# niessner/BundleFusion

Measured on AMD Instinct MI355X. Metric: frames/sec end-to-end (SIFT+SBA+TSDF re-integrate), 640x480 @4mm, higher is better.
Workload: dtype f32

## Files before the change

### bundlefusion_amd/csrc/solver.hip

```cpp
#include <hip/hip_runtime.h>

#include <algorithm>
#include <cstring>
#include <vector>

#include "bf_device.h"
#include "bf_resources.h"
#include "bf_se3.h"

using namespace bf;

namespace {

constexpr float FLOAT_EPSILON = 0.000001f;
constexpr uint32_t NOSLOT = 0xFFFFFFFFu;
constexpr int DENSE_BLK = 120;

typedef float f32x4 __attribute__((ext_vector_type(4)));

enum Flag { FL_DONE = 0, FL_NUM_SLOTS = 1, FL_NUM_PAIRS = 2, FL_LIST_LEN = 3, FL_GN_ITERS = 4, FL_BARRIER_FAIL = 5, FL_SLOT_OVERFLOW = 6, FL_PCG_ITERS = 8, FL_COUNT = 40 };

struct Cfg {
    float denseDistThresh, denseNormalThresh, denseColorThresh, denseColorGradientMin, denseDepthMin, denseDepthMax;
    uint32_t subsample;
// ... 523 lines not shown
            d.slotG[(size_t)s * 6 + (lane - 36)] = c.wSparse * accD + dD;
        } else if (lane < 46) {
            d.slotP[(size_t)s * 4 + (lane - 42)] = accD;
        }
    }
}

__global__ __launch_bounds__(256) void k_rows(Dev d) {
    if (d.flags[FL_DONE]) return;
    const uint32_t lane = threadIdx.x & 63;
    const uint32_t i = blockIdx.x * (blockDim.x >> 6) + (threadIdx.x >> 6);
    if (i >= d.N) return;
    const uint32_t s0 = d.rowStart[i], s1 = d.rowStart[i + 1];
    float acc = 0.0f;
    for (uint32_t s = s0; s < s1; ++s) {
        if (lane < 36) acc += d.slotD[(size_t)s * 36 + lane];
        else if (lane < 42) acc += d.slotG[(size_t)s * 6 + (lane - 36)];
        else if (lane < 46) acc += d.slotP[(size_t)s * 4 + (lane - 42)];
    }
    if (lane < 36) d.diagA[(size_t)i * 36 + lane] = acc;
    else if (lane < 42) d.rhs[(size_t)i * 6 + (lane - 36)] = -acc;
    else if (lane < 45) d.prec[(size_t)i * 6 + 3 + (lane - 42)] = acc > FLOAT_EPSILON ? 1.0f / acc : 1.0f;
    else if (lane == 45) {
        const float v = acc > FLOAT_EPSILON ? 1.0f / acc : 1.0f;
        d.prec[(size_t)i * 6 + 0] = v; d.prec[(size_t)i * 6 + 1] = v; d.prec[(size_t)i * 6 + 2] = v;
    }
}

BF_DEV float blockSum(float v, float* sh) {
    v = wave_sum(v);
    __syncthreads();
    if ((threadIdx.x & 63) == 0) sh[threadIdx.x >> 6] = v;
    __syncthreads();
    float t = 0.0f;
    for (uint32_t w = 0; w < (blockDim.x >> 6); ++w) t += sh[w];
    return t;
}
BF_DEV float blockMax(float v, float* sh) {
    v = wave_max(v);
    __syncthreads();
    if ((threadIdx.x & 63) == 0) sh[threadIdx.x >> 6] = v;
    __syncthreads();
    float t = 0.0f;
    for (uint32_t w = 0; w < (blockDim.x >> 6); ++w) t = fmaxf(t, sh[w]);
    return t;
}

constexpr size_t PCG_LDS_MAX = 160 * 1024 - 1024;
template <bool VEC_LDS>
__global__ __launch_bounds__(1024) void k_pcg(Dev d, uint32_t nLin, uint32_t gnIter, int lastGN) {
    if (d.flags[FL_DONE]) return;
    extern __shared__ float dynLds[];
    __shared__ float sh[16];
    const uint32_t N = d.N, n6 = 6 * N;
    const uint32_t lane = threadIdx.x & 63, wave = threadIdx.x >> 6, nWaves = blockDim.x >> 6;
    float* const P = VEC_LDS ? dynLds : d.p;
    float* const R = VEC_LDS ? dynLds + n6 : d.r;
    float* const X = VEC_LDS ? dynLds + 2 * n6 : d.delta;
    float* const AP = VEC_LDS ? dynLds + 3 * n6 : d.Ap;
    const float* const M = VEC_LDS ? dynLds + 4 * n6 : d.prec;
    const uint32_t* const RS = VEC_LDS ? (const uint32_t*)(dynLds + 5 * n6) : d.rowStart;
    if (VEC_LDS) {
        for (uint32_t t = threadIdx.x; t < n6; t += blockDim.x) dynLds[4 * n6 + t] = d.prec[t];
        for (uint32_t t = threadIdx.x; t <= N; t += blockDim.x) ((uint32_t*)(dynLds + 5 * n6))[t] = d.rowStart[t];
        __syncthreads();
    }
    float part = 0.0f;
    for (uint32_t t = threadIdx.x; t < n6; t += blockDim.x) {
        const bool var = t >= 6;
        const float rr = var ? d.rhs[t] : 0.0f;
        const float pp = var ? M[t] * rr : 0.0f;
        R[t] = rr; P[t] = pp; X[t] = 0.0f;
        part += rr * pp;
    }
    float rzOld = blockSum(part, sh);
    uint32_t it = 0;
    for (uint32_t lin = 0; lin < nLin; ++lin) {
        bool last = (lin == nLin - 1);
        ++it;
        __syncthreads();
        {
            const uint32_t q = lane >> 4, l16 = lane & 15;
            for (uint32_t i0 = 1; i0 < N; i0 += 4 * nWaves) {
                const uint32_t i = i0 + wave * 4 + q;
                float acc[6] = {0, 0, 0, 0, 0, 0};
                if (i < N) {
                    const uint32_t s0 = RS[i], s1 = RS[i + 1];
                    for (uint32_t s = s0 + l16; s < s1; s += 16) {
                        const float4* O4 = reinterpret_cast<const float4*>(d.slotO + (size_t)s * 36);
                        const uint32_t col = d.slotCol[s];
                        float O[36];
#pragma unroll
                        for (int v = 0; v < 9; ++v) { const float4 o = O4[v]; O[4 * v] = o.x; O[4 * v + 1] = o.y; O[4 * v + 2] = o.z; O[4 * v + 3] = o.w; }
                        const float* pj = P + 6 * col;
                        const float q0 = pj[0], q1 = pj[1], q2 = pj[2], q3 = pj[3], q4 = pj[4], q5 = pj[5];
#pragma unroll
                        for (int a = 0; a < 6; ++a)
                            acc[a] += ((((O[a * 6 + 0] * q0 + O[a * 6 + 1] * q1) + O[a * 6 + 2] * q2) + O[a * 6 + 3] * q3) + O[a * 6 + 4] * q4) + O[a * 6 + 5] * q5;
                    }
                }
#pragma unroll
                for (int a = 0; a < 6; ++a)
#pragma unroll
                    for (int o = 8; o > 0; o >>= 1) acc[a] += __shfl_xor(acc[a], o, 64);
                if (i < N && l16 < 6) {
                    const float* A = d.diagA + (size_t)i * 36 + l16 * 6;
                    const float* pi = P + 6 * i;
                    float v = 0.0f;
#pragma unroll
                    for (int b = 0; b < 6; ++b) v += A[b] * pi[b];
                    float sel = acc[0];
                    if (l16 == 1) sel = acc[1]; else if (l16 == 2) sel = acc[2]; else if (l16 == 3) sel = acc[3]; else if (l16 == 4) sel = acc[4]; else if (l16 == 5) sel = acc[5];
                    AP[6 * i + l16] = v + sel;
                }
            }
        }
        __syncthreads();
        part = 0.0f;
        for (uint32_t t = 6 + threadIdx.x; t < n6; t += blockDim.x) part += P[t] * AP[t];
        const float pAp = blockSum(part, sh);
        const float alpha = pAp > FLOAT_EPSILON ? rzOld / pAp : 0.0f;
        part = 0.0f;
        for (uint32_t t = 6 + threadIdx.x; t < n6; t += blockDim.x) {
            X[t] = X[t] + alpha * P[t];
            const float rr = R[t] - alpha * AP[t];
            R[t] = rr;
            part += (M[t] * rr) * rr;
        }
        const float rzNew = blockSum(part, sh);
        if (fabsf(pAp) < 5e-7f) last = true;
        const float beta = rzOld > FLOAT_EPSILON ? rzNew / rzOld : 0.0f;
        rzOld = rzNew;
        for (uint32_t t = 6 + threadIdx.x; t < n6; t += blockDim.x) P[t] = M[t] * R[t] + beta * P[t];
        if (last) break;
    }
    __syncthreads();
    float mx = 0.0f;
    for (uint32_t i = 1 + threadIdx.x; i < N; i += blockDim.x) {
        const f3 dT = ld3(X + 6 * i), dW = ld3(X + 6 * i + 3);
        f3 nw, nt;
        lieUpdate(dW, dT, ld3(d.xRot + 3 * i), ld3(d.xTrans + 3 * i), nw, nt);
        d.xRot[3 * i] = nw.x; d.xRot[3 * i + 1] = nw.y; d.xRot[3 * i + 2] = nw.z;
        d.xTrans[3 * i] = nt.x; d.xTrans[3 * i + 1] = nt.y; d.xTrans[3 * i + 2] = nt.z;
        if (d.valid[i] != 0) mx = fmaxf(mx, fmaxf(fmaxf(fmaxf(fabsf(dW.x), fabsf(dT.x)), fmaxf(fabsf(dW.y), fabsf(dT.y))), fmaxf(fabsf(dW.z), fabsf(dT.z))));
    }
    mx = blockMax(mx, sh);
    if (threadIdx.x == 0) {
        d.flags[FL_GN_ITERS] = (int)gnIter + 1;
        d.flags[FL_PCG_ITERS + gnIter] = (int)it;
        if (!lastGN && mx < 0.005f) d.flags[FL_DONE] = 1;
    }
}

constexpr uint32_t COOP_THREADS = 256, COOP_THREADS_SMALL = 1024, COOP_MAX_GROUPS = 64, COOP_ROWS_PER_GROUP = 8, COOP_SPIN_LIMIT = 1u << 22;

BF_DEV void coopPublish(float* p, float v) { __hip_atomic_store(p, v, __ATOMIC_RELAXED, __HIP_MEMORY_SCOPE_AGENT); }
BF_DEV float coopRead(const float* p) { return __hip_atomic_load(p, __ATOMIC_RELAXED, __HIP_MEMORY_SCOPE_AGENT); }

BF_DEV bool gridBarrier(uint32_t* counter, uint32_t target, int* shFail) {
    __builtin_amdgcn_s_waitcnt(0);
    __syncthreads();
    if (threadIdx.x == 0) {
        __hip_atomic_fetch_add(counter, 1u, __ATOMIC_RELAXED, __HIP_MEMORY_SCOPE_AGENT);
        uint32_t spins = 0;
        while (__hip_atomic_load(counter, __ATOMIC_RELAXED, __HIP_MEMORY_SCOPE_AGENT) < target) {
            __builtin_amdgcn_s_sleep(2);
            if (++spins > COOP_SPIN_LIMIT) { *shFail = 1; break; }
        }
    }
    __syncthreads();
    return *shFail == 0;
}

template <uint32_t THREADS>
__global__ __launch_bounds__(THREADS) void k_pcg_coop(Dev d, uint32_t nLin, uint32_t gnIter, int lastGN, uint32_t ldsFloats, uint32_t vecGlobal) {
    if (d.flags[FL_DONE]) return;
    extern __shared__ __align__(16) float coopLds[];
    float* const dynLds = coopLds;
    __shared__ float sh[16];
    __shared__ int shFail;
    const uint32_t N = d.N, n6 = 6 * N, G = gridDim.x;
    const uint32_t lane = threadIdx.x & 63, wave = threadIdx.x >> 6, nWaves = THREADS >> 6;
    const uint32_t vecFloats = (5 * n6 + (N + 1) + 3) & ~3u;
    float* const vec = vecGlobal ? d.coopVec + (size_t)blockIdx.x * vecFloats : dynLds;
    float* const P = vec;
    float* const R = vec + n6;
    float* const X = vec + 2 * n6;
    float* const AP = vec + 3 * n6;
    float* const M = vec + 4 * n6;
    uint32_t* const RS = reinterpret_cast<uint32_t*>(vec + 5 * n6);
    const uint32_t rpg = (N - 1 + G - 1) / G;
    const uint32_t r0 = min(N, 1 + blockIdx.x * rpg), r1 = min(N, r0 + rpg);
    const uint32_t ldsBase = vecGlobal ? 0u : 5 * n6 + (N + 1);
    float* const DG = dynLds + ldsBase;
    float* const OL = dynLds + ((ldsBase + rpg * 36 + 3) & ~3u);
    if (threadIdx.x == 0) shFail = 0;
    for (uint32_t t = threadIdx.x; t < n6; t += THREADS) M[t] = d.prec[t];
    for (uint32_t t = threadIdx.x; t <= N; t += THREADS) RS[t] = d.rowStart[t];
    for (uint32_t t = threadIdx.x; t < (r1 - r0) * 36; t += THREADS) DG[t] = d.diagA[(size_t)r0 * 36 + t];
    __syncthreads();
    const uint32_t sBase = RS[r0], sEnd = RS[r1];
    const uint32_t ldsSlots = min(sEnd - sBase, (ldsFloats - (uint32_t)(OL - dynLds)) / 37u);
    uint32_t* const CL = reinterpret_cast<uint32_t*>(OL + (size_t)ldsSlots * 36);
    {
        const float4* src = reinterpret_cast<const float4*>(d.slotO + (size_t)sBase * 36);
        float4* dst = reinterpret_cast<float4*>(OL);
        for (uint32_t t = threadIdx.x; t < ldsSlots * 9; t += THREADS) dst[t] = src[t];
        for (uint32_t t = threadIdx.x; t < ldsSlots; t += THREADS) CL[t] = d.slotCol[sBase + t];
    }
    float part = 0.0f;
    for (uint32_t t = threadIdx.x; t < n6; t += THREADS) {
        const bool var = t >= 6;
        const float rr = var ? d.rhs[t] : 0.0f;
        const float pp = var ? M[t] * rr : 0.0f;
        R[t] = rr; P[t] = pp; X[t] = 0.0f;
        part += rr * pp;
    }
    float rzOld = blockSum(part, sh);
    float* const xchg[2] = {d.Ap, d.p};
    uint32_t* const counter = reinterpret_cast<uint32_t*>(d.gridBar) + gnIter;
    uint32_t it = 0;
    for (uint32_t lin = 0; lin < nLin; ++lin) {
        bool last = (lin == nLin - 1);
        ++it;
        __syncthreads();
        float* const out = G > 1 ? xchg[lin & 1] : AP;
        {
            const uint32_t g8 = lane >> 3, a = lane & 7;
            for (uint32_t i = r0 + wave; i < r1; i += nWaves) {
                const uint32_t s0 = RS[i], s1 = RS[i + 1];
                float acc = 0.0f;
                if (a < 6) {
                    for (uint32_t s = s0 + g8; s < s1; s += 8) {
                        const uint32_t ls = s - sBase;
                        float o0, o1, o2, o3, o4, o5; uint32_t col;
                        if (ls < ldsSlots) {
                            const float* O = OL + (size_t)ls * 36 + a * 6;
                            o0 = O[0]; o1 = O[1]; o2 = O[2]; o3 = O[3]; o4 = O[4]; o5 = O[5]; col = CL[ls];
                        } else {
                            const float* O = d.slotO + (size_t)s * 36 + a * 6;
                            o0 = O[0]; o1 = O[1]; o2 = O[2]; o3 = O[3]; o4 = O[4]; o5 = O[5]; col = d.slotCol[s];
                        }
                        const float* pj = P + 6 * col;
                        acc += ((((o0 * pj[0] + o1 * pj[1]) + o2 * pj[2]) + o3 * pj[3]) + o4 * pj[4]) + o5 * pj[5];
                    }
                }
                acc += __shfl_xor(acc, 8, 64); acc += __shfl_xor(acc, 16, 64); acc += __shfl_xor(acc, 32, 64);
                if (lane < 6) {
                    const float* A = DG + (size_t)(i - r0) * 36 + lane * 6;
                    const float* pi = P + 6 * i;
                    float v = 0.0f;
#pragma unroll
                    for (int b = 0; b < 6; ++b) v += A[b] * pi[b];
                    if (G > 1) coopPublish(out + 6 * i + lane, v + acc); else out[6 * i + lane] = v + acc;
                }
            }
        }
        part = 0.0f;
        if (G > 1) {
            if (!gridBarrier(counter, G * it, &shFail)) { if (threadIdx.x == 0) d.flags[FL_BARRIER_FAIL] = 1; return; }
            for (uint32_t t = 6 + threadIdx.x; t < n6; t += THREADS) { const float ap = coopRead(out + t); AP[t] = ap; part += P[t] * ap; }
        } else {
            __syncthreads();
            for (uint32_t t = 6 + threadIdx.x; t < n6; t += THREADS) part += P[t] * AP[t];
        }
        const float pAp = blockSum(part, sh);
        const float alpha = pAp > FLOAT_EPSILON ? rzOld / pAp : 0.0f;
        part = 0.0f;
        for (uint32_t t = 6 + threadIdx.x; t < n6; t += THREADS) {
            X[t] = X[t] + alpha * P[t];
            const float rr = R[t] - alpha * AP[t];
            R[t] = rr;
            part += (M[t] * rr) * rr;
        }
        const float rzNew = blockSum(part, sh);
        if (fabsf(pAp) < 5e-7f) last = true;
        const float beta = rzOld > FLOAT_EPSILON ? rzNew / rzOld : 0.0f;
        rzOld = rzNew;
        for (uint32_t t = 6 + threadIdx.x; t < n6; t += THREADS) P[t] = M[t] * R[t] + beta * P[t];
        if (last) break;
    }
    if (blockIdx.x != 0) return;
    __syncthreads();
    float mx = 0.0f;
    for (uint32_t i = 1 + threadIdx.x; i < N; i += THREADS) {
        const f3 dT = ld3(X + 6 * i), dW = ld3(X + 6 * i + 3);
        f3 nw, nt;
        lieUpdate(dW, dT, ld3(d.xRot + 3 * i), ld3(d.xTrans + 3 * i), nw, nt);
        d.xRot[3 * i] = nw.x; d.xRot[3 * i + 1] = nw.y; d.xRot[3 * i + 2] = nw.z;
        d.xTrans[3 * i] = nt.x; d.xTrans[3 * i + 1] = nt.y; d.xTrans[3 * i + 2] = nt.z;
        if (d.valid[i] != 0) mx = fmaxf(mx, fmaxf(fmaxf(fmaxf(fabsf(dW.x), fabsf(dT.x)), fmaxf(fabsf(dW.y), fabsf(dT.y))), fmaxf(fabsf(dW.z), fabsf(dT.z))));
    }
    mx = blockMax(mx, sh);
    if (threadIdx.x == 0) {
        d.flags[FL_GN_ITERS] = (int)gnIter + 1;
        d.flags[FL_PCG_ITERS + gnIter] = (int)it;
        if (!lastGN && mx < 0.005f) d.flags[FL_DONE] = 1;
    }
}

BF_DEV float absMaxResidual(const Dev& d, const bf_entry_j& e, float w) {
    if (!validCorr(e)) return 0.0f;
    const m44 TI = poseToMatrix(ld3(d.xRot + 3 * e.imgIdx_i), ld3(d.xTrans + 3 * e.imgIdx_i));
    const m44 TJ = poseToMatrix(ld3(d.xRot + 3 * e.imgIdx_j), ld3(d.xTrans + 3 * e.imgIdx_j));
    const f3 a = xform(TI, mk3(e.pos_i[0], e.pos_i[1], e.pos_i[2])), b = xform(TJ, mk3(e.pos_j[0], e.pos_j[1], e.pos_j[2]));
    return fmaxf(w * fabsf(a.z - b.z), fmaxf(w * fabsf(a.x - b.x), w * fabsf(a.y - b.y)));
}

constexpr uint32_t MAXRES_GROUPS = 64;
BF_DEV bool maxResBetter(float o, int oi, float cur, int ci) { return cur < o || (cur == o && oi < ci && o > 0.0f); }

__global__ __launch_bounds__(1024) void k_max_residual(Dev d, float w) {
    __shared__ float sv[1024];
    __shared__ int si[1024];
    float best = 0.0f; int bi = 0;
    for (uint32_t c = blockIdx.x * blockDim.x + threadIdx.x; c < d.C; c += gridDim.x * blockDim.x) {
        const float r = absMaxResidual(d, d.corr[c], w);
        if (best < r) { best = r; bi = (int)c; }
    }
    sv[threadIdx.x] = best; si[threadIdx.x] = bi;
    __syncthreads();
    for (uint32_t s = blockDim.x >> 1; s > 0; s >>= 1) {
        if (threadIdx.x < s) {
            const float o = sv[threadIdx.x + s]; const int oi = si[threadIdx.x + s];
            if (maxResBetter(o, oi, sv[threadIdx.x], si[threadIdx.x])) { sv[threadIdx.x] = o; si[threadIdx.x] = oi; }
        }
        __syncthreads();
    }
    if (threadIdx.x == 0) { d.maxResPart[blockIdx.x] = sv[0]; d.maxIdxPart[blockIdx.x] = si[0]; }
}

__global__ __launch_bounds__(64) void k_max_residual_final(Dev d, uint32_t G) {
    float best = 0.0f; int bi = 0;
    if (threadIdx.x < G) { best = d.maxResPart[threadIdx.x]; bi = d.maxIdxPart[threadIdx.x]; }
#pragma unroll
    for (int o = 32; o > 0; o >>= 1) {
        const float ov = __shfl_xor(best, o, 64); const int oi = __shfl_xor(bi, o, 64);
        if (maxResBetter(ov, oi, best, bi)) { best = ov; bi = oi; }
    }
    if (threadIdx.x == 0) { d.maxRes[0] = best; d.maxIdx[0] = bi; }
}

__global__ void k_count_high(Dev d, float w, float thresh) {
    const uint32_t c = blockIdx.x * blockDim.x + threadIdx.x;
    bool hi = false;
    if (c < d.C) hi = absMaxResidual(d, d.corr[c], w) > thresh;
    const unsigned long long m = __ballot(hi);
    if ((threadIdx.x & 63) == 0 && m) atomicAdd(d.highCount, __popcll(m));
}

__global__ __launch_bounds__(1024) void k_energy(Dev d, float w, uint32_t slot, int honourDone) {
    if (honourDone && d.flags[FL_DONE] && slot > (uint32_t)d.flags[FL_GN_ITERS]) return;
    __shared__ float sh[16];
    float part = 0.0f;
    for (uint32_t c = threadIdx.x; c < d.C; c += blockDim.x) {
        const bf_entry_j e = d.corr[c];
        if (!validCorr(e)) continue;
        const m44 TI = poseToMatrix(ld3(d.xRot + 3 * e.imgIdx_i), ld3(d.xTrans + 3 * e.imgIdx_i));
        const m44 TJ = poseToMatrix(ld3(d.xRot + 3 * e.imgIdx_j), ld3(d.xTrans + 3 * e.imgIdx_j));
        const f3 r = xform(TI, mk3(e.pos_i[0], e.pos_i[1], e.pos_i[2])) - xform(TJ, mk3(e.pos_j[0], e.pos_j[1], e.pos_j[2]));
        part += w * dot3(r, r);
    }
    const float tot = blockSum(part, sh);
    if (threadIdx.x == 0) d.energies[slot] = tot;
}

__global__ void k_matrices_to_poses(const m44* T, uint32_t n, float* rot3, float* trans3, const int* valid) {
    const uint32_t i = blockIdx.x * blockDim.x + threadIdx.x;
    if (i < n && valid[i]) {
        f3 r, t;
        matrixToPose(T[i], r, t);
        rot3[3 * i] = r.x; rot3[3 * i + 1] = r.y; rot3[3 * i + 2] = r.z;
        trans3[3 * i] = t.x; trans3[3 * i + 1] = t.y; trans3[3 * i + 2] = t.z;
    }
}
__global__ void k_poses_to_matrices(const float* rot3, const float* trans3, uint32_t n, m44* T, const int* valid) {
    const uint32_t i = blockIdx.x * blockDim.x + threadIdx.x;
    if (i < n && valid[i]) T[i] = poseToMatrix(ld3(rot3 + 3 * i), ld3(trans3 + 3 * i));
}

__global__ void k_expand_dense(Dev d, float* JtJ, float* Jtr) {
    const uint32_t nPairs = (uint32_t)d.flags[FL_NUM_PAIRS];
    const uint32_t dim = 6 * d.N;
    for (uint32_t p = 0; p < nPairs; ++p) {
        const uint2 pr = d.densePairs[p];
        const float* blk = d.denseBlocks + (size_t)p * DENSE_BLK;
        const uint32_t t = threadIdx.x;
        if (t < 36) {
            const uint32_t a = t / 6, b = t % 6;
            JtJ[(size_t)(pr.x * 6 + a) * dim + pr.x * 6 + b] += blk[a * 6 + b];
            JtJ[(size_t)(pr.y * 6 + a) * dim + pr.y * 6 + b] += blk[36 + a * 6 + b];
            JtJ[(size_t)(pr.x * 6 + a) * dim + pr.y * 6 + b] += blk[72 + a * 6 + b];
            JtJ[(size_t)(pr.y * 6 + b) * dim + pr.x * 6 + a] += blk[72 + a * 6 + b];
        } else if (t < 42) {
            Jtr[pr.x * 6 + (t - 36)] += blk[108 + (t - 36)];
            Jtr[pr.y * 6 + (t - 36)] += blk[114 + (t - 36)];
        }
        __syncthreads();
    }
}

}

struct bf_solver {
    bf_solver_config cfg;
    uint32_t maxImages, maxResiduals, maxCorrPerImage;
    Dev d{};
    hipStream_t stream = nullptr;
    bf::Resources res;
    std::vector<float> convergence;
    float hMaxRes = 0.0f; int hMaxIdx = 0; int hBarrierFail = 0;
    bool pcgWide = true;
    int pcgGroups = -1;
    uint32_t maxCoopGroups = COOP_MAX_GROUPS;
    bool forceVecGlobal = false;
    size_t coopVecFloats = 0;
    uint32_t lastN = 0, lastGNrequested = 0;
    float lastWeightSparse = 1.0f;
    bool lastUsedDense = false;
};

extern "C" {

int bf_solver_create(uint32_t maxNumberOfImages, uint32_t maxNumResiduals, const bf_solver_config* cfg, bf_solver** out) {
    BF_REQUIRE(cfg && out, "null argument");
    BF_REQUIRE(maxNumberOfImages >= 2 && maxNumResiduals > 0, "bad capacity");
    bf_solver* s = new bf_solver();
    bf::CreateGuard<bf_solver> guard(s, bf_solver_destroy);
    s->cfg = *cfg;
    s->maxImages = maxNumberOfImages; s->maxResiduals = maxNumResiduals;
    BF_HIP_TRY(hipFuncSetAttribute(reinterpret_cast<const void*>(&k_pcg<true>), hipFuncAttributeMaxDynamicSharedMemorySize, (int)PCG_LDS_MAX));
    BF_HIP_TRY(hipFuncSetAttribute(reinterpret_cast<const void*>(&k_pcg_coop<COOP_THREADS>), hipFuncAttributeMaxDynamicSharedMemorySize, (int)PCG_LDS_MAX));
    BF_HIP_TRY(hipFuncSetAttribute(reinterpret_cast<const void*>(&k_pcg_coop<COOP_THREADS_SMALL>), hipFuncAttributeMaxDynamicSharedMemorySize, (int)PCG_LDS_MAX));
    if (const char* e = getenv("BF_PCG_WIDE")) s->pcgWide = atoi(e) != 0;
    if (const char* e = getenv("BF_PCG_GROUPS")) s->pcgGroups = atoi(e);
    if (const char* e = getenv("BF_PCG_VEC_GLOBAL")) s->forceVecGlobal = atoi(e) != 0;
    {
        int dev = 0, cus = 0;
        if (hipGetDevice(&dev) == hipSuccess && hipDeviceGetAttribute(&cus, hipDeviceAttributeMultiprocessorCount, dev) == hipSuccess && cus > 0)
            s->maxCoopGroups = std::max(1u, std::min(COOP_MAX_GROUPS, (uint32_t)cus / 2u));
        else (void)hipGetLastError();
    }
    s->maxCorrPerImage = std::min(std::max(maxNumResiduals / maxNumberOfImages, 1000u), 4000u);
    const size_t N = maxNumberOfImages, M = N * N, C = maxNumResiduals;
    Dev& d = s->d;
    d.maxSlots = (uint32_t)std::min<size_t>(M, 2 * C + (N <= 64 ? M : 4 * N));
    d.maxPairs = (uint32_t)(N * (N - 1) / 2);
    if (N > 64) d.maxPairs = (uint32_t)std::min<size_t>(d.maxPairs, d.maxSlots);
    s->coopVecFloats = ((31 * N + 4096 <= PCG_LDS_MAX / 4 && !s->forceVecGlobal) ? (size_t)4 : (size_t)s->maxCoopGroups * ((31 * N + 1 + 3) & ~(size_t)3));
    bf::Resources& R = s->res;
    BF_TRY(R.device(&d.T, N)); BF_TRY(R.device(&d.Tinv, N)); BF_TRY(R.device(&d.keyCount, M)); BF_TRY(R.device(&d.keyStart, M)); BF_TRY(R.device(&d.cursor, M));
    BF_TRY(R.device(&d.slotOfKey, M)); BF_TRY(R.device(&d.denseRaw, M)); BF_TRY(R.device(&d.keyPair, M)); BF_TRY(R.device(&d.rowStart, N + 1));
    BF_TRY(R.device(&d.slotCol, (size_t)d.maxSlots)); BF_TRY(R.device(&d.slotKey, (size_t)d.maxSlots)); BF_TRY(R.device(&d.corrList, 2 * C));
    BF_TRY(R.device(&d.slotD, (size_t)d.maxSlots * 36)); BF_TRY(R.device(&d.slotO, (size_t)d.maxSlots * 36)); BF_TRY(R.device(&d.slotG, (size_t)d.maxSlots * 6));
    BF_TRY(R.device(&d.slotP, (size_t)d.maxSlots * 4)); BF_TRY(R.device(&d.diagA, N * 36)); BF_TRY(R.device(&d.rhs, N * 6)); BF_TRY(R.device(&d.prec, N * 6));
    BF_TRY(R.device(&d.delta, N * 6)); BF_TRY(R.device(&d.r, N * 6)); BF_TRY(R.device(&d.p, N * 6)); BF_TRY(R.device(&d.Ap, N * 6));
    BF_TRY(R.device(&d.densePairs, (size_t)d.maxPairs)); BF_TRY(R.device(&d.denseWeight, (size_t)d.maxPairs));
    BF_TRY(R.device(&d.denseBlocks, (size_t)d.maxPairs * DENSE_BLK)); BF_TRY(R.device(&d.flags, FL_COUNT)); BF_TRY(R.device(&d.gridBar, 32)); BF_TRY(R.device(&d.energies, 40));
    BF_TRY(R.device(&d.maxRes, 1)); BF_TRY(R.device(&d.maxIdx, 1)); BF_TRY(R.device(&d.highCount, 1)); BF_TRY(R.device(&d.numEntriesPerRow, N));
    BF_TRY(R.device(&d.scanRow, 3 * (N + 1))); BF_TRY(R.device(&d.coopVec, s->coopVecFloats)); BF_TRY(R.device(&d.maxResPart, MAXRES_GROUPS)); BF_TRY(R.device(&d.maxIdxPart, MAXRES_GROUPS));
    (void)hipMemset(d.flags, 0, FL_COUNT * sizeof(int));
    *out = guard.dismiss();
    return BF_OK;
}

int bf_solver_destroy(bf_solver* s) {
    if (!s) return BF_OK;
    (void)hipStreamSynchronize(s->stream);
    delete s;
    return BF_OK;
}

int bf_solver_set_stream(bf_solver* s, void* st) { BF_REQUIRE(s, "null solver"); s->stream = (hipStream_t)st; return BF_OK; }

int bf_solver_solve(bf_solver* s, bf_entry_j* d_corr, uint32_t numCorr, const int32_t* d_valid, uint32_t N, uint32_t nNonLin, uint32_t nLin,
                    const bf_cached_frame* d_cache, uint32_t cw, uint32_t ch, const float K4[4], const float* wS, const float* wDD,
                    const float* wDC, uint32_t numWeights, int usePairwise, float* d_rot, float* d_trans, int rebuildJT, int findMaxResidual,
                    uint32_t revalidateIdx) {
    (void)rebuildJT; (void)revalidateIdx;
    BF_REQUIRE(s && d_valid && d_rot && d_trans && wS && wDD && wDC, "null argument");
    BF_REQUIRE(numCorr == 0 || d_corr, "null correspondences");
    nNonLin = std::min(nNonLin, numWeights);
    BF_REQUIRE(N > 1 && nNonLin > 0 && nLin > 0, "numberOfImages > 1 && nNonLinearIterations > 0 required");
    BF_REQUIRE(N <= s->maxImages && numCorr <= s->maxResiduals, "problem exceeds the solver's capacity");
    BF_REQUIRE(nNonLin <= 32, "at most 32 non-linear iterations");
    Dev d = s->d;
    d.corr = d_corr; d.C = numCorr; d.valid = d_valid; d.N = N; d.xRot = d_rot; d.xTrans = d_trans; d.cache = d_cache;
    s->d = d;
    Cfg c;
    c.denseDistThresh = s->cfg.denseDistThresh; c.denseNormalThresh = s->cfg.denseNormalThresh; c.denseColorThresh = s->cfg.denseColorThresh;
    c.denseColorGradientMin = s->cfg.denseColorGradientMin; c.denseDepthMin = s->cfg.denseDepthMin; c.denseDepthMax = s->cfg.denseDepthMax;
    c.subsample = s->cfg.denseOverlapCheckSubsampleFactor;
    c.W = cw; c.H = ch;
    if (d_cache) {
        BF_REQUIRE(K4, "cache intrinsics missing");
        BF_REQUIRE(c.subsample > 0 && cw / c.subsample > 8, "denseDepthWidth / subsample factor must exceed 8");
        BF_REQUIRE((cw / c.subsample) * (ch / c.subsample) <= 512, "overlap pre-filter samples exceed one workgroup");
        c.fx = K4[0]; c.fy = K4[1]; c.cx = K4[2]; c.cy = K4[3];
    } else { c.fx = c.fy = c.cx = c.cy = 0.0f; }
    c.usePairwise = usePairwise;
    hipStream_t st = s->stream;
    const size_t M = (size_t)N * N;
    hipLaunchKernelGGL(k_solve_begin, dim3(1), dim3(64), 0, st, d);
    const bool record = s->cfg.recordConvergence != 0;
    if (record) hipLaunchKernelGGL(k_energy, dim3(1), dim3(1024), 0, st, d, wS[0], 0u, 0);
    bool anyDense = false, prevDense = false;
    for (uint32_t it = 0; it < nNonLin; ++it) {
        c.wSparse = wS[it]; c.wDepth = wDD[it]; c.wColor = wDC[it];
        const int useDense = (d_cache != nullptr) && (c.wDepth > 0.0f || c.wColor > 0.0f);
        anyDense |= useDense != 0;
        const bool reuse = it > 0 && !useDense && !prevDense;
        prevDense = useDense != 0;
        hipLaunchKernelGGL(k_poses, dim3(std::max<uint32_t>(div_up(N, 256), std::min<uint32_t>(div_up((uint32_t)M, 256), 128u))), dim3(256), 0, st, d, reuse ? 0u : (uint32_t)M, useDense);
        if (useDense) {
            const dim3 grid = usePairwise ? dim3(N, N) : dim3(N - 1, 1);
            hipLaunchKernelGGL(k_dense_overlap, grid, dim3(512), 0, st, d, c);
        }
        if (!reuse) {
            if (numCorr) hipLaunchKernelGGL(k_key_count, dim3(div_up(numCorr, 256)), dim3(256), 0, st, d);
            if (it == 0) hipLaunchKernelGGL(k_row_entries, dim3(div_up(N, 64)), dim3(64), 0, st, d);
            hipLaunchKernelGGL(k_scan_rows, dim3(N), dim3(64), 0, st, d, useDense);
            hipLaunchKernelGGL(k_scan_base, dim3(1), dim3(1024), 0, st, d);
            hipLaunchKernelGGL(k_scan_fill, dim3(N), dim3(64), 0, st, d, useDense);
            if (numCorr) hipLaunchKernelGGL(k_fill, dim3(div_up(numCorr, 256)), dim3(256), 0, st, d);
        }
        if (useDense) {
            const uint32_t g = std::min<uint32_t>(std::max<uint32_t>(N * (N - 1) / 2, 1u), 1024u);
            hipLaunchKernelGGL(k_dense_weight, dim3(g), dim3(256), 0, st, d, c);
            hipLaunchKernelGGL(k_dense_build, dim3(g), dim3(256), 0, st, d, c);
        }
        hipLaunchKernelGGL(k_slots, dim3(std::min<uint32_t>(div_up(d.maxSlots, 4), 2048u)), dim3(256), 0, st, d, c, useDense);
        hipLaunchKernelGGL(k_rows, dim3(div_up(N, 4)), dim3(256), 0, st, d);
        {
            uint32_t G = N <= 32 ? 1u : std::min(s->maxCoopGroups, div_up(N - 1, COOP_ROWS_PER_GROUP));
            if (s->pcgGroups > 0) G = std::min(std::min<uint32_t>((uint32_t)s->pcgGroups, N - 1), s->maxCoopGroups);
            const uint32_t rpg = div_up(N - 1, G);
            size_t baseFloats = ((size_t)31 * N + 1 + (size_t)rpg * 36 + 3) & ~(size_t)3;
            const uint32_t vecGlobal = (s->forceVecGlobal || baseFloats + 37 * 8 > PCG_LDS_MAX / 4) ? 1u : 0u;
            if (vecGlobal) baseFloats = ((size_t)rpg * 36 + 3) & ~(size_t)3;
            const size_t ldsFloats = std::min<size_t>(PCG_LDS_MAX / 4, baseFloats + (size_t)rpg * std::min<uint32_t>(N - 1, 96u) * 37);
            const bool vecFits = !vecGlobal || (size_t)G * (((size_t)31 * N + 1 + 3) & ~(size_t)3) <= s->coopVecFloats;
            if (s->pcgGroups != 0 && nNonLin <= 32 && vecFits && baseFloats + 37 * 8 <= PCG_LDS_MAX / 4)
            {
                if (s->pcgWide && G == 1 && 6 * N <= COOP_THREADS)
                    hipLaunchKernelGGL(k_pcg_coop<COOP_THREADS_SMALL>, dim3(G), dim3(COOP_THREADS_SMALL), ldsFloats * 4, st, d, nLin, it, (int)(it == nNonLin - 1), (uint32_t)ldsFloats, vecGlobal);
                else
                    hipLaunchKernelGGL(k_pcg_coop<COOP_THREADS>, dim3(G), dim3(COOP_THREADS), ldsFloats * 4, st, d, nLin, it, (int)(it == nNonLin - 1), (uint32_t)ldsFloats, vecGlobal);
            }
            else if ((size_t)N * 124 + 4 <= PCG_LDS_MAX)
                hipLaunchKernelGGL(k_pcg<true>, dim3(1), dim3(1024), (size_t)N * 124 + 4, st, d, nLin, it, (int)(it == nNonLin - 1));
            else hipLaunchKernelGGL(k_pcg<false>, dim3(1), dim3(1024), 0, st, d, nLin, it, (int)(it == nNonLin - 1));
        }
        if (record) hipLaunchKernelGGL(k_energy, dim3(1), dim3(1024), 0, st, d, c.wSparse, it + 1, 1);
    }
    BF_HIP_TRY(hipGetLastError());
    s->lastN = N; s->lastGNrequested = nNonLin; s->lastWeightSparse = wS[nNonLin - 1]; s->lastUsedDense = anyDense;
    if (findMaxResidual) {
        if (s->lastWeightSparse > 0.0f && numCorr > 0) {
            const uint32_t gmr = std::min<uint32_t>(MAXRES_GROUPS, std::max<uint32_t>(1u, div_up(numCorr, 1024u)));
            hipLaunchKernelGGL(k_max_residual, dim3(gmr), dim3(1024), 0, st, d, s->lastWeightSparse);
            hipLaunchKernelGGL(k_max_residual_final, dim3(1), dim3(64), 0, st, d, gmr);
            BF_HIP_TRY(hipMemcpyAsync(&s->hMaxRes, d.maxRes, 4, hipMemcpyDeviceToHost, st));
            BF_HIP_TRY(hipMemcpyAsync(&s->hMaxIdx, d.maxIdx, 4, hipMemcpyDeviceToHost, st));
            BF_HIP_TRY(hipMemcpyAsync(&s->hBarrierFail, d.flags + FL_BARRIER_FAIL, 4, hipMemcpyDeviceToHost, st));
            BF_HIP_TRY(hipStreamSynchronize(st));
            BF_REQUIRE(s->hBarrierFail == 0, "PCG grid barrier timed out (a workgroup of k_pcg_coop was never scheduled)");
        } else { s->hMaxRes = 0.0f; s->hMaxIdx = 0; }
    }
    if (record) {
        int flags[FL_COUNT];
        float en[40];
        BF_HIP_TRY(hipMemcpyAsync(flags, d.flags, sizeof flags, hipMemcpyDeviceToHost, st));
        BF_HIP_TRY(hipMemcpyAsync(en, d.energies, sizeof en, hipMemcpyDeviceToHost, st));
        BF_HIP_TRY(hipStreamSynchronize(st));
        s->convergence.assign(nNonLin + 1, -1.0f);
        for (int k = 0; k <= flags[FL_GN_ITERS] && k <= (int)nNonLin; ++k) s->convergence[k] = en[k];
    }
    return BF_OK;
}

int bf_solver_get_var_to_corr_num_entries_per_row(bf_solver* s, const int32_t** d_out) {
    BF_REQUIRE(s && d_out, "null argument");
    *d_out = s->d.numEntriesPerRow;
    return BF_OK;
}

int bf_solver_get_corr_overflow(bf_solver* s, uint32_t* numImagesOverLimit, uint32_t* limit) {
    BF_REQUIRE(s && numImagesOverLimit, "null argument");
    if (limit) *limit = s->maxCorrPerImage;
    *numImagesOverLimit = 0;
    const uint32_t N = s->lastN;
    if (N == 0) return BF_OK;
    std::vector<int> rows(N);
    BF_HIP_TRY(hipMemcpyAsync(rows.data(), s->d.numEntriesPerRow, sizeof(int) * N, hipMemcpyDeviceToHost, s->stream));
    BF_HIP_TRY(hipStreamSynchronize(s->stream));
    for (int r : rows) if ((uint32_t)std::max(r, 0) > s->maxCorrPerImage) (*numImagesOverLimit)++;
    return BF_OK;
}

int bf_solver_get_max_residual(bf_solver* s, float* mx, int32_t* idx) {
    BF_REQUIRE(s && mx && idx, "null argument");
    *mx = s->hMaxRes; *idx = s->hMaxIdx;
    return BF_OK;
}

int bf_solver_get_max_residual_pair(bf_solver* s, uint32_t curFrame, const bf_entry_j* d_corr, uint32_t imageIndices[2], float* maxRes, int* remove) {
    (void)curFrame;
    BF_REQUIRE(s && d_corr && imageIndices && maxRes && remove, "null argument");
    bf_entry_j e;
    BF_HIP_TRY(hipMemcpyAsync(&e, d_corr + s->hMaxIdx, sizeof e, hipMemcpyDeviceToHost, s->stream));
    BF_HIP_TRY(hipStreamSynchronize(s->stream));
    imageIndices[0] = e.imgIdx_i; imageIndices[1] = e.imgIdx_j;
    *maxRes = s->hMaxRes;
    *remove = (!(e.imgIdx_i == 0 && e.imgIdx_j < 10) && s->hMaxRes > s->cfg.optMaxResThresh) ? 1 : 0;
    return BF_OK;
}

int bf_solver_use_verification(bf_solver* s, const bf_entry_j* d_corr, uint32_t numCorr, int* out) {
    BF_REQUIRE(s && d_corr && out && numCorr > 0, "bad argument");
    BF_REQUIRE(s->d.xRot && s->d.xTrans, "useVerification before solve");
    Dev d = s->d;
    d.corr = d_corr; d.C = numCorr;
    BF_HIP_TRY(hipMemsetAsync(d.highCount, 0, 4, s->stream));
    hipLaunchKernelGGL(k_count_high, dim3(div_up(numCorr, 256)), dim3(256), 0, s->stream, d, 1.0f, s->cfg.verifyOptDistThresh);
    int cnt = 0;
    BF_HIP_TRY(hipMemcpyAsync(&cnt, d.highCount, 4, hipMemcpyDeviceToHost, s->stream));
    BF_HIP_TRY(hipStreamSynchronize(s->stream));
    *out = ((float)cnt / (float)numCorr >= s->cfg.verifyOptPercentThresh) ? 1 : 0;
    return BF_OK;
}

int bf_solver_get_convergence(bf_solver* s, float* out, uint32_t cap, uint32_t* count) {
    BF_REQUIRE(s && out && count, "null argument");
    const uint32_t n = (uint32_t)std::min<size_t>(cap, s->convergence.size());
    for (uint32_t i = 0; i < n; ++i) out[i] = s->convergence[i];
    *count = n;
    return BF_OK;
}

int bf_solver_get_iteration_counts(bf_solver* s, int32_t* out, uint32_t cap) {
    BF_REQUIRE(s && out && cap > 0, "bad argument");
    int flags[FL_COUNT];
    BF_HIP_TRY(hipMemcpyAsync(flags, s->d.flags, sizeof flags, hipMemcpyDeviceToHost, s->stream));
    BF_HIP_TRY(hipStreamSynchronize(s->stream));
    BF_REQUIRE(flags[FL_BARRIER_FAIL] == 0, "PCG grid barrier timed out (a workgroup of k_pcg_coop was never scheduled)");
    out[0] = flags[FL_GN_ITERS];
    for (uint32_t k = 1; k < cap && k <= 32; ++k) out[k] = (int)k <= flags[FL_GN_ITERS] ? flags[FL_PCG_ITERS + k - 1] : 0;
    return BF_OK;
}

int bf_solver_debug_dense_system(bf_solver* s, float* hJtJ, float* hJtr, uint32_t N, int32_t* numPairs) {
    BF_REQUIRE(s && hJtJ && hJtr && numPairs && N == s->lastN, "bad argument");
    const size_t dim = 6 * (size_t)N;
    float *dJ = nullptr, *dr = nullptr;
    bf::Resources scratch;
    BF_TRY(scratch.device(&dJ, dim * dim));
    BF_TRY(scratch.device(&dr, dim));
    BF_HIP_TRY(hipMemsetAsync(dJ, 0, dim * dim * 4, s->stream));
    BF_HIP_TRY(hipMemsetAsync(dr, 0, dim * 4, s->stream));
    if (s->lastUsedDense) hipLaunchKernelGGL(k_expand_dense, dim3(1), dim3(64), 0, s->stream, s->d, dJ, dr);
    BF_HIP_TRY(hipMemcpyAsync(hJtJ, dJ, dim * dim * 4, hipMemcpyDeviceToHost, s->stream));
    BF_HIP_TRY(hipMemcpyAsync(hJtr, dr, dim * 4, hipMemcpyDeviceToHost, s->stream));
    int flags[FL_COUNT];
    BF_HIP_TRY(hipMemcpyAsync(flags, s->d.flags, sizeof flags, hipMemcpyDeviceToHost, s->stream));
    BF_HIP_TRY(hipStreamSynchronize(s->stream));
    *numPairs = s->lastUsedDense ? flags[FL_NUM_PAIRS] : 0;
    return BF_OK;
}

int bf_solver_debug_system(bf_solver* s, float* hA, float* hb, float* hPrec, uint32_t N) {
    BF_REQUIRE(s && hA && hb && hPrec && N == s->lastN, "bad argument");
    const size_t dim = 6 * (size_t)N;
    hipStream_t st = s->stream;
    std::vector<uint32_t> rowStart(N + 1);
    BF_HIP_TRY(hipMemcpyAsync(rowStart.data(), s->d.rowStart, (N + 1) * sizeof(uint32_t), hipMemcpyDeviceToHost, st));
    BF_HIP_TRY(hipStreamSynchronize(st));
    const uint32_t nSlots = rowStart[N];
    std::vector<uint32_t> col(std::max<uint32_t>(nSlots, 1));
    std::vector<float> O((size_t)std::max<uint32_t>(nSlots, 1) * 36), D((size_t)N * 36);
    if (nSlots) {
        BF_HIP_TRY(hipMemcpyAsync(col.data(), s->d.slotCol, nSlots * sizeof(uint32_t), hipMemcpyDeviceToHost, st));
        BF_HIP_TRY(hipMemcpyAsync(O.data(), s->d.slotO, (size_t)nSlots * 36 * sizeof(float), hipMemcpyDeviceToHost, st));
    }
    BF_HIP_TRY(hipMemcpyAsync(D.data(), s->d.diagA, D.size() * sizeof(float), hipMemcpyDeviceToHost, st));
    BF_HIP_TRY(hipMemcpyAsync(hb, s->d.rhs, dim * sizeof(float), hipMemcpyDeviceToHost, st));
    BF_HIP_TRY(hipMemcpyAsync(hPrec, s->d.prec, dim * sizeof(float), hipMemcpyDeviceToHost, st));
    BF_HIP_TRY(hipStreamSynchronize(st));
    std::fill(hA, hA + dim * dim, 0.0f);
    for (uint32_t i = 0; i < N; ++i) {
        for (uint32_t a = 0; a < 6; ++a)
            for (uint32_t b = 0; b < 6; ++b) hA[(6 * i + a) * dim + 6 * i + b] += D[(size_t)i * 36 + a * 6 + b];
        for (uint32_t sl = rowStart[i]; sl < rowStart[i + 1]; ++sl)
            for (uint32_t a = 0; a < 6; ++a)
                for (uint32_t b = 0; b < 6; ++b) hA[(6 * i + a) * dim + 6 * (size_t)col[sl] + b] += O[(size_t)sl * 36 + a * 6 + b];
    }
    return BF_OK;
}

// ... 24 lines not shown
```

Baseline: 1461.

## Add wave-replicated single-block PCG kernel for small problems

Replaces the 1024-thread cooperative PCG path for small problems (6N <= 256) with a specialized kernel. In it, every wave holds a private copy of the search direction in LDS and does dot products with DPP/permlane wave reductions instead of block-wide reductions. This cuts per-iteration block barriers to one and keeps off-diagonal blocks in registers or LDS. The kernel is templated on the number of 64-lane chunks. It adds redundant reduction work per wave and a new code path that is only taken when the wide option is enabled and vectors fit in LDS.

```diff
diff --git a/bundlefusion_amd/csrc/solver.hip b/bundlefusion_amd/csrc/solver.hip
--- a/bundlefusion_amd/csrc/solver.hip
+++ b/bundlefusion_amd/csrc/solver.hip
@@ -699,7 +699,7 @@
     }
 }
 
-constexpr uint32_t COOP_THREADS = 256, COOP_THREADS_SMALL = 1024, COOP_MAX_GROUPS = 64, COOP_ROWS_PER_GROUP = 8, COOP_SPIN_LIMIT = 1u << 22;
+constexpr uint32_t COOP_THREADS = 256, COOP_MAX_GROUPS = 64, COOP_ROWS_PER_GROUP = 8, COOP_SPIN_LIMIT = 1u << 22;
 
 BF_DEV void coopPublish(float* p, float v) { __hip_atomic_store(p, v, __ATOMIC_RELAXED, __HIP_MEMORY_SCOPE_AGENT); }
 BF_DEV float coopRead(const float* p) { return __hip_atomic_load(p, __ATOMIC_RELAXED, __HIP_MEMORY_SCOPE_AGENT); }
@@ -846,6 +846,184 @@
     }
 }
 
+constexpr uint32_t SMALL_MAX_WAVES = 16, SMALL_TRIPS = 3, SMALL_VEC = 256;
+static_assert(SMALL_MAX_WAVES * SMALL_TRIPS * 6 >= COOP_THREADS - 6 && SMALL_VEC >= COOP_THREADS, "every row of a 6 N <= 256 problem has a wave and a trip");
+
+template <int CTRL> BF_DEV float dppMov(float v) { return __builtin_bit_cast(float, __builtin_amdgcn_mov_dpp(__builtin_bit_cast(int, v), CTRL, 0xF, 0xF, true)); }
+template <int O> BF_DEV float laneXor(float v) {
+    if constexpr (O == 1) return dppMov<0xB1>(v);
+    else if constexpr (O == 2) return dppMov<0x4E>(v);
+    else if constexpr (O == 4) return dppMov<0x1B>(dppMov<0x141>(v));
+    else if constexpr (O == 8) return dppMov<0x128>(v);
+    else if constexpr (O == 16) {
+        const uint32_t u = __builtin_bit_cast(uint32_t, v);
+        const auto r = __builtin_amdgcn_permlane16_swap(u, u, false, false);
+        return __builtin_bit_cast(float, (threadIdx.x & 16) ? r[0] : r[1]);
+    } else {
+        static_assert(O == 32, "lane distance");
+        const uint32_t u = __builtin_bit_cast(uint32_t, v);
+        const auto r = __builtin_amdgcn_permlane32_swap(u, u, false, false);
+        return __builtin_bit_cast(float, (threadIdx.x & 32) ? r[0] : r[1]);
+    }
+}
+BF_DEV float waveSumAlu(float v) {
+    v += laneXor<32>(v); v += laneXor<16>(v); v += laneXor<8>(v); v += laneXor<4>(v); v += laneXor<2>(v); v += laneXor<1>(v);
+    return v;
+}
+
+template <uint32_t NJ>
+__global__ __launch_bounds__(SMALL_MAX_WAVES * 64) void k_pcg_small(Dev d, uint32_t nLin, uint32_t gnIter, int lastGN, uint32_t ldsFloats) {
+    if (d.flags[FL_DONE]) return;
+    extern __shared__ __align__(16) float smallLds[];
+    const uint32_t N = d.N, n6 = 6 * N;
+    const uint32_t lane = threadIdx.x & 63, wave = threadIdx.x >> 6, nWaves = blockDim.x >> 6;
+    float* const PW = smallLds + wave * SMALL_VEC;
+    float* const APB = smallLds + nWaves * SMALL_VEC;
+    float* const OL = APB + 2 * SMALL_VEC;
+    const uint32_t g8 = lane >> 3, a = lane & 7;
+    uint32_t rowI[SMALL_TRIPS], sNext[SMALL_TRIPS], sStop[SMALL_TRIPS], col0[SMALL_TRIPS];
+    float o0[SMALL_TRIPS][6], dg[SMALL_TRIPS][6];
+    bool more = false;
+#pragma unroll
+    for (uint32_t k = 0; k < SMALL_TRIPS; ++k) {
+        const uint32_t i = 1 + wave + k * nWaves;
+        rowI[k] = i; sNext[k] = sStop[k] = 0; col0[k] = 0;
+#pragma unroll
+        for (int b = 0; b < 6; ++b) { o0[k][b] = 0.0f; dg[k][b] = 0.0f; }
+        if (i < N) {
+            const uint32_t s = d.rowStart[i] + g8, s1 = d.rowStart[i + 1];
+            if (a < 6 && s < s1) {
+                const float* O = d.slotO + (size_t)s * 36 + a * 6;
+#pragma unroll
+                for (int b = 0; b < 6; ++b) o0[k][b] = O[b];
+                col0[k] = d.slotCol[s];
+                sNext[k] = s + 8; sStop[k] = s1;
+                more |= s + 8 < s1;
+            }
+            if (lane < 6) {
+                const float* A = d.diagA + (size_t)i * 36 + lane * 6;
+#pragma unroll
+                for (int b = 0; b < 6; ++b) dg[k][b] = A[b];
+            }
+        }
+    }
+    const uint32_t sBase = d.rowStart[1], sEnd = d.rowStart[N];
+    const bool longRows = __syncthreads_or(more) != 0;
+    const uint32_t ldsSlots = longRows ? min(sEnd - sBase, (ldsFloats - (uint32_t)(OL - smallLds)) / 37u) : 0u;
+    uint32_t* const CL = reinterpret_cast<uint32_t*>(OL + (size_t)ldsSlots * 36);
+    {
+        const float4* src = reinterpret_cast<const float4*>(d.slotO + (size_t)sBase * 36);
+        float4* dst = reinterpret_cast<float4*>(OL);
+        for (uint32_t t = threadIdx.x; t < ldsSlots * 9; t += blockDim.x) dst[t] = src[t];
+        for (uint32_t t = threadIdx.x; t < ldsSlots; t += blockDim.x) CL[t] = d.slotCol[sBase + t];
+    }
+    bool own[NJ];
+    float m[NJ], r[NJ], x[NJ], p[NJ], ap[NJ];
+#pragma unroll
+    for (uint32_t j = 0; j < NJ; ++j) {
+        const uint32_t t = 6 + 64 * j + lane;
+        own[j] = t < n6;
+        m[j] = own[j] ? d.prec[t] : 0.0f;
+        r[j] = own[j] ? d.rhs[t] : 0.0f;
+        p[j] = m[j] * r[j]; x[j] = 0.0f;
+        if (own[j]) PW[t] = p[j];
+    }
+    if (lane < 6) PW[lane] = 0.0f;
+    float rzOld = 0.0f;
+#pragma unroll
+    for (uint32_t j = 0; j < (NJ < 4 ? NJ + 1 : 4); ++j) {
+        const uint32_t t = 64 * j + lane;
+        const bool var = t >= 6 && t < n6;
+        const float rr = var ? d.rhs[t] : 0.0f;
+        const float pp = var ? d.prec[t] * rr : 0.0f;
+        rzOld += waveSumAlu(0.0f + rr * pp);
+    }
+    __syncthreads();
+    uint32_t it = 0;
+    for (uint32_t lin = 0; lin < nLin; ++lin) {
+        bool last = (lin == nLin - 1);
+        ++it;
+        float* const out = APB + (lin & 1) * SMALL_VEC;
+#pragma unroll
+        for (uint32_t k = 0; k < SMALL_TRIPS; ++k) {
+            const uint32_t i = rowI[k];
+            if (i >= N) break;
+            const float* pj = PW + 6 * col0[k];
+            float acc = 0.0f;
+            acc += ((((o0[k][0] * pj[0] + o0[k][1] * pj[1]) + o0[k][2] * pj[2]) + o0[k][3] * pj[3]) + o0[k][4] * pj[4]) + o0[k][5] * pj[5];
+            if (longRows) {
+                uint32_t s = sNext[k];
+                const uint32_t s1 = sStop[k], sLds = min(s1, sBase + ldsSlots);
+                for (; s < sLds; s += 8) {
+                    const uint32_t ls = s - sBase;
+                    const float* O = OL + (size_t)ls * 36 + a * 6;
+                    const float* q = PW + 6 * CL[ls];
+                    acc += ((((O[0] * q[0] + O[1] * q[1]) + O[2] * q[2]) + O[3] * q[3]) + O[4] * q[4]) + O[5] * q[5];
+                }
+                for (; s < s1; s += 8) {
+                    const float* O = d.slotO + (size_t)s * 36 + a * 6;
+                    const float* q = PW + 6 * d.slotCol[s];
+                    acc += ((((O[0] * q[0] + O[1] * q[1]) + O[2] * q[2]) + O[3] * q[3]) + O[4] * q[4]) + O[5] * q[5];
+                }
+            }
+            acc += laneXor<8>(acc); acc += laneXor<16>(acc); acc += laneXor<32>(acc);
+            const float* pi = PW + 6 * i;
+            float v = 0.0f;
+#pragma unroll
+            for (int b = 0; b < 6; ++b) v += dg[k][b] * pi[b];
+            if (lane < 6) out[6 * i + lane] = v + acc;
+        }
+        __syncthreads();
+        float pAp = 0.0f;
+#pragma unroll
+        for (uint32_t j = 0; j < NJ; ++j) ap[j] = out[6 + 64 * j + lane];
+#pragma unroll
+        for (uint32_t j = 0; j < NJ; ++j) {
+            ap[j] = own[j] ? ap[j] : 0.0f;
+            pAp += waveSumAlu(0.0f + p[j] * ap[j]);
+        }
+        const float alpha = pAp > FLOAT_EPSILON ? rzOld / pAp : 0.0f;
+        float rzNew = 0.0f;
+#pragma unroll
+        for (uint32_t j = 0; j < NJ; ++j) {
+            const float xx = x[j] + alpha * p[j];
+            const float rr = r[j] - alpha * ap[j];
+            x[j] = own[j] ? xx : 0.0f; r[j] = own[j] ? rr : 0.0f;
+            rzNew += waveSumAlu(0.0f + (m[j] * r[j]) * r[j]);
+        }
+        if (fabsf(pAp) < 5e-7f) last = true;
+        const float beta = rzOld > FLOAT_EPSILON ? rzNew / rzOld : 0.0f;
+        rzOld = rzNew;
+#pragma unroll
+        for (uint32_t j = 0; j < NJ; ++j) {
+            const float pp = m[j] * r[j] + beta * p[j];
+            p[j] = own[j] ? pp : 0.0f;
+            if (own[j]) PW[6 + 64 * j + lane] = p[j];
+        }
+        if (last) break;
+    }
+    if (wave != 0) return;
+#pragma unroll
+    for (uint32_t j = 0; j < NJ; ++j) if (own[j]) PW[6 + 64 * j + lane] = x[j];
+    const float* const X = PW;
+    float mx = 0.0f;
+    const uint32_t i = 1 + lane;
+    if (i < N) {
+        const f3 dT = ld3(X + 6 * i), dW = ld3(X + 6 * i + 3);
+        f3 nw, nt;
+        lieUpdate(dW, dT, ld3(d.xRot + 3 * i), ld3(d.xTrans + 3 * i), nw, nt);
+        d.xRot[3 * i] = nw.x; d.xRot[3 * i + 1] = nw.y; d.xRot[3 * i + 2] = nw.z;
+        d.xTrans[3 * i] = nt.x; d.xTrans[3 * i + 1] = nt.y; d.xTrans[3 * i + 2] = nt.z;
+        if (d.valid[i] != 0) mx = fmaxf(mx, fmaxf(fmaxf(fmaxf(fabsf(dW.x), fabsf(dT.x)), fmaxf(fabsf(dW.y), fabsf(dT.y))), fmaxf(fabsf(dW.z), fabsf(dT.z))));
+    }
+    mx = fmaxf(0.0f, wave_max(mx));
+    if (lane == 0) {
+        d.flags[FL_GN_ITERS] = (int)gnIter + 1;
+        d.flags[FL_PCG_ITERS + gnIter] = (int)it;
+        if (!lastGN && mx < 0.005f) d.flags[FL_DONE] = 1;
+    }
+}
+
 BF_DEV float absMaxResidual(const Dev& d, const bf_entry_j& e, float w) {
     if (!validCorr(e)) return 0.0f;
     const m44 TI = poseToMatrix(ld3(d.xRot + 3 * e.imgIdx_i), ld3(d.xTrans + 3 * e.imgIdx_i));
@@ -978,7 +1156,10 @@
     s->maxImages = maxNumberOfImages; s->maxResiduals = maxNumResiduals;
     BF_HIP_TRY(hipFuncSetAttribute(reinterpret_cast<const void*>(&k_pcg<true>), hipFuncAttributeMaxDynamicSharedMemorySize, (int)PCG_LDS_MAX));
     BF_HIP_TRY(hipFuncSetAttribute(reinterpret_cast<const void*>(&k_pcg_coop<COOP_THREADS>), hipFuncAttributeMaxDynamicSharedMemorySize, (int)PCG_LDS_MAX));
-    BF_HIP_TRY(hipFuncSetAttribute(reinterpret_cast<const void*>(&k_pcg_coop<COOP_THREADS_SMALL>), hipFuncAttributeMaxDynamicSharedMemorySize, (int)PCG_LDS_MAX));
+    BF_HIP_TRY(hipFuncSetAttribute(reinterpret_cast<const void*>(&k_pcg_small<1>), hipFuncAttributeMaxDynamicSharedMemorySize, (int)PCG_LDS_MAX));
+    BF_HIP_TRY(hipFuncSetAttribute(reinterpret_cast<const void*>(&k_pcg_small<2>), hipFuncAttributeMaxDynamicSharedMemorySize, (int)PCG_LDS_MAX));
+    BF_HIP_TRY(hipFuncSetAttribute(reinterpret_cast<const void*>(&k_pcg_small<3>), hipFuncAttributeMaxDynamicSharedMemorySize, (int)PCG_LDS_MAX));
+    BF_HIP_TRY(hipFuncSetAttribute(reinterpret_cast<const void*>(&k_pcg_small<4>), hipFuncAttributeMaxDynamicSharedMemorySize, (int)PCG_LDS_MAX));
     if (const char* e = getenv("BF_PCG_WIDE")) s->pcgWide = atoi(e) != 0;
     if (const char* e = getenv("BF_PCG_GROUPS")) s->pcgGroups = atoi(e);
     if (const char* e = getenv("BF_PCG_VEC_GLOBAL")) s->forceVecGlobal = atoi(e) != 0;
@@ -1089,8 +1270,19 @@
             const bool vecFits = !vecGlobal || (size_t)G * (((size_t)31 * N + 1 + 3) & ~(size_t)3) <= s->coopVecFloats;
             if (s->pcgGroups != 0 && nNonLin <= 32 && vecFits && baseFloats + 37 * 8 <= PCG_LDS_MAX / 4)
             {
-                if (s->pcgWide && G == 1 && 6 * N <= COOP_THREADS)
-                    hipLaunchKernelGGL(k_pcg_coop<COOP_THREADS_SMALL>, dim3(G), dim3(COOP_THREADS_SMALL), ldsFloats * 4, st, d, nLin, it, (int)(it == nNonLin - 1), (uint32_t)ldsFloats, vecGlobal);
+                if (s->pcgWide && G == 1 && 6 * N <= COOP_THREADS && !vecGlobal) {
+                    const uint32_t waves = std::min(SMALL_MAX_WAVES, std::max(8u, 4u * div_up(div_up(N - 1, SMALL_TRIPS), 4u)));
+                    const size_t smallBase = (size_t)(waves + 2) * SMALL_VEC;
+                    const uint32_t smallLds = (uint32_t)std::min<size_t>(PCG_LDS_MAX / 4, smallBase + std::max<size_t>(8, (size_t)(N - 1) * (N - 1) * 37));
+                    const dim3 block(waves * 64);
+                    const int lastGN = (int)(it == nNonLin - 1);
+                    switch (div_up(6 * N - 6, 64)) {
+                        case 1: hipLaunchKernelGGL(k_pcg_small<1>, dim3(1), block, smallLds * 4, st, d, nLin, it, lastGN, smallLds); break;
+                        case 2: hipLaunchKernelGGL(k_pcg_small<2>, dim3(1), block, smallLds * 4, st, d, nLin, it, lastGN, smallLds); break;
+                        case 3: hipLaunchKernelGGL(k_pcg_small<3>, dim3(1), block, smallLds * 4, st, d, nLin, it, lastGN, smallLds); break;
+                        default: hipLaunchKernelGGL(k_pcg_small<4>, dim3(1), block, smallLds * 4, st, d, nLin, it, lastGN, smallLds); break;
+                    }
+                }
                 else
                     hipLaunchKernelGGL(k_pcg_coop<COOP_THREADS>, dim3(G), dim3(COOP_THREADS), ldsFloats * 4, st, d, nLin, it, (int)(it == nNonLin - 1), (uint32_t)ldsFloats, vecGlobal);
             }
```

After: 1516, median of 6. +3.8%, better.
